# wbuntine/libstb

Measured on AMD Instinct MI355X. Metric: S-table cells/s, higher is better.
Workload: dtype f64

## Files before the change

include/stb_hip.h:

```cpp
#ifndef STB_HIP_H
#define STB_HIP_H

#include <stddef.h>
#include <stdint.h>

#ifdef __cplusplus
extern "C" {
#endif

const char *stb_last_error(void);
int stb_device_count(void);
int stb_device_name(char *buf, int len);

int stb_set_device(int dev);
int stb_get_device(void);
int stb_device_enter(int dev);
void stb_device_leave(int prev);

void *stb_device_malloc(size_t bytes);
void stb_device_free(void *p);
void *stb_host_malloc(size_t bytes);
void stb_host_free(void *p);
void *stb_host_malloc_huge(size_t bytes);
void stb_host_free_huge(void *p);
// ... 158 lines not shown
  double grad, delta;
} stb_modea_info_t;
int stb_groups_aterms_grad(stb_groups_t *g, const double *x_host, int D, double *val_out, double *grad_out);
int stb_groups_modea(stb_groups_t *g, double a_lo, double a_hi, double tol, int rounds_max, double *a_hat, double *curv,
                     stb_modea_info_t *info);
int stb_groups_update_restaurants(stb_groups_t *g, const uint32_t *T, const double *bpar);
int stb_groups_pairs_begin(stb_groups_t *g);
int stb_groups_pairs_put(stb_groups_t *g, const uint32_t *n, const uint16_t *t, uint64_t count, unsigned *maxn, unsigned *maxt);
int stb_groups_pairs_put_ragged(stb_groups_t *g, int I, const int *K, uint32_t *const *n, uint16_t *const *t, unsigned *maxn, unsigned *maxt);
int stb_groups_pairs_commit(stb_groups_t *g, const uint32_t *T, const double *bpar, unsigned N, unsigned M);
int stb_groups_update_pairs(stb_groups_t *g, const uint32_t *nflat, const uint16_t *tflat);
unsigned stb_groups_fallbacks(void);
int stb_grid_shape(unsigned N, unsigned M, int D, int *C_out, int *G_out, int *K_out);
int stb_groups_shape(const stb_groups_t *g, int *I, uint64_t *G, unsigned *N, unsigned *M, int *Dmax);
int stb_groups_last_form(const stb_groups_t *g, int *fused, int *which, int *sparse, int *C, int *R);
int stb_groups_aterms_timed(stb_groups_t *g, const double *x_host, int D, double *out_host,
                            float *ms_fill, float *ms_sweep, float *ms_terms);

int stb_sample_tcounts(const double *d_table, const double *d_S1, unsigned N, unsigned M, double a,
                       const double *d_bpar, int I, const uint64_t *d_koff , const uint32_t *d_n,
                       uint16_t *d_t, uint32_t *d_T, const double *d_h ,
                       uint64_t seed, uint64_t sweep, void *stream);
typedef struct stb_tcounts stb_tcounts_t;
stb_tcounts_t *stb_tcounts_create(int I, const int *K, const uint32_t *nflat, const uint16_t *tflat,
                                  const double *hflat, unsigned M );
int stb_tcounts_set_h(stb_tcounts_t *s, const double *hflat);
int stb_tcounts_sweep(stb_tcounts_t *s, double a, const double *bpar ,
                      uint64_t seed, uint64_t sweep, int nsweeps);
int stb_tcounts_get(stb_tcounts_t *s, uint16_t *t_out, uint32_t *T_out);
int stb_tcounts_to_groups(stb_tcounts_t *s, stb_groups_t *g, const double *bpar );
// ... 74 lines not shown
```

libstb_amd/capi.py:

```python
from __future__ import annotations

import ctypes as C
import os
from functools import lru_cache

import numpy as np

_HERE = os.path.dirname(os.path.abspath(__file__))
LIB_PATH = os.environ.get("STB_LIB_PATH") or os.path.join(_HERE, "lib", "libstb_amd.so")

S_STABLE, S_UVTABLE, S_FLOAT, S_VERBOSE, S_QUITONBOUND, S_THREADS, S_ASYMPT = 1, 2, 4, 8, 16, 32, 64
FILL_SCALED, FILL_LOGDOMAIN, FILL_SCALED_STEP, FILL_SPLIT, FILL_FUSED, FILL_PC, FILL_CHAIN, FILL_CHAINX, FILL_CK, FILL_HB = 0, 1, 2, 3, 4, 5, 6, 7, 8, 9

c_double_p = C.POINTER(C.c_double)
c_u32_p = C.POINTER(C.c_uint32)
c_u16_p = C.POINTER(C.c_uint16)
c_int_p = C.POINTER(C.c_int)
c_float_p = C.POINTER(C.c_float)

LOGDENS = C.CFUNCTYPE(C.c_double, C.c_double, C.c_void_p)
GETVAL = C.CFUNCTYPE(None, c_u32_p, c_u16_p, C.c_uint, C.c_uint)


class StbError(RuntimeError):
# ... 34 lines not shown
    if not os.path.exists(LIB_PATH):
        raise StbError(
            f"{LIB_PATH} is missing: build it with `python -c 'import __graft_entry__ as g; g.build()'` "
            "or `make -C libstb_amd/csrc` (there is no pure-Python or CPU implementation)")
    try:
        import torch
    except Exception:
        pass
    L = C.CDLL(LIB_PATH)
    u, d, i, vp, u64, sz = C.c_uint, C.c_double, C.c_int, C.c_void_p, C.c_uint64, C.c_size_t

    ROUND5 = {"stb_groups_pairs_begin", "stb_groups_pairs_put", "stb_groups_pairs_put_ragged", "stb_groups_pairs_commit",
              "stb_groups_update_pairs", "stb_groups_fallbacks", "stb_grid_shape", "stb_bterms_update",
              "stb_table_probe", "stb_slow_launches", "stb_shared_gpu_mode", "stb_set_shared_gpu", "stb_note_launch_span",
              "stb_lookup_V", "stb_lookup_U", "stb_lookup_UV", "stb_groups_aterms_multi", "stb_groups_create_node",
              "stb_groups_last_form"}

    def sig(name, res, args):
        try:
            f = getattr(L, name)
        except AttributeError:
            if name in ROUND5 and os.environ.get("STB_LIB_PATH"):
                return
            raise
        f.restype = res
        f.argtypes = args

    sig("S_make", vp, [u, u, u, u, d, C.c_uint32])
    sig("S_tag", None, [vp, C.c_char_p])
    sig("S_remake", i, [vp, d])
    sig("S_free", None, [vp])
# ... 65 lines not shown
    sig("stb_groups_aterms_async", i, [vp, c_double_p, i, c_double_p, vp])
    sig("stb_groups_wait", i, [vp])
    sig("stb_groups_aterms_multi", i, [C.POINTER(vp), i, c_double_p, i, c_double_p])
    sig("stb_groups_create_node", i, [i, i, c_int_p, c_u32_p, c_u32_p, c_u16_p, c_double_p, u, u, i, C.POINTER(vp)])
    sig("stb_groups_aterms_device", i, [vp, c_double_p, i, vp, vp])
    sig("stb_groups_update_restaurants", i, [vp, c_u32_p, c_double_p])
    sig("stb_groups_pairs_begin", i, [vp])
    sig("stb_groups_pairs_put", i, [vp, c_u32_p, c_u16_p, u64, C.POINTER(u), C.POINTER(u)])
    sig("stb_groups_pairs_put_ragged", i, [vp, i, c_int_p, vp, vp, C.POINTER(u), C.POINTER(u)])
    sig("stb_groups_pairs_commit", i, [vp, c_u32_p, c_double_p, u, u])
    sig("stb_groups_update_pairs", i, [vp, c_u32_p, c_u16_p])
    sig("stb_groups_fallbacks", C.c_uint, [])
    sig("stb_grid_shape", i, [u, u, i, c_int_p, c_int_p, c_int_p])
    sig("stb_groups_shape", i, [vp, c_int_p, C.POINTER(u64), C.POINTER(u), C.POINTER(u), c_int_p])
    sig("stb_groups_last_form", i, [vp, c_int_p, c_int_p, c_int_p, c_int_p, c_int_p])
    sig("stb_sampler_cache_clear", None, [])
    sig("stb_groups_aterms_timed", i, [vp, c_double_p, i, c_double_p, c_float_p, c_float_p, c_float_p])
    sig("stb_sample_tcounts", i, [vp, vp, u, u, d, vp, i, vp, vp, vp, vp, vp, u64, u64, vp])
    sig("stb_tcounts_create", vp, [i, c_int_p, c_u32_p, c_u16_p, c_double_p, u])
    sig("stb_tcounts_set_h", i, [vp, c_double_p])
    sig("stb_tcounts_sweep", i, [vp, d, c_double_p, u64, u64, i])
    sig("stb_tcounts_get", i, [vp, c_u16_p, c_u32_p])
    sig("stb_tcounts_to_groups", i, [vp, vp, c_double_p])
    sig("stb_tcounts_free", None, [vp])
    sig("stb_sample_tcounts_window", i, [vp, vp, u, u, d, vp, i, vp, vp, vp, vp, vp, u, u, u64, u64, vp])
    sig("stb_tcounts_sweep_window", i, [vp, d, c_double_p, u, u, u64, u64, i])
    sig("stb_sample_tindic", i, [vp, u, u, d, vp, i, vp, vp, vp, vp, vp, vp, vp, u, u64, u64, vp])
    sig("stb_tindic_create", vp, [i, c_int_p, c_u32_p, c_u16_p, c_double_p, c_u32_p, u, u])
    sig("stb_tindic_set_h", i, [vp, c_double_p])
    sig("stb_tindic_sweep", i, [vp, d, c_double_p, u64, u64, i])
# ... 709 lines not shown
```

libstb_amd/csrc/grid_hb.hip:

```cpp
#include <mutex>
#include <vector>

#include "fill_chain.h"

#define GH_PMAX 7
#define GH_NWMAX 8
#define GH_MAXR 48
#define GH_SL 4
#define GH_FSL 4
#define GH_EOFF32 (1u << 30)
#define GH_WRITTEN 0x8000000000000000ull
#define GH_SPIN 48
#define GH_MAXPH 16
#define GH_JOB_MB 192
#define GH_JOBS 1500
#define GH_JQ 64
#define GH_JNUM (GH_JQ + 1)
#define GH_JBASE 128
#define GH_PB(C) ((C) == 8 ? 9 : 8)
#ifndef GH_NOSTORE
#define GH_NOSTORE 0
#endif

struct gh_args {
  const double *a;
  const double2 *lt;
  unsigned *hdr;
  unsigned *ticket;
  unsigned long long *ck_v;
  unsigned *ck_e;
  double *state_v;
  int *state_e;
  const unsigned *tile_off;
  const unsigned *tinfo;
// ... 39 lines not shown
}

template <int C>
__device__ __forceinline__ void gh_row(double (&v)[C], double (&coef)[C], double s) {
  const double t0 = wave_shr1_zero(v[C - 1]) * s;
#pragma unroll
  for (int i = C - 1; i >= 1; i--) v[i] = fma(coef[i], v[i], v[i - 1]);
  v[0] = fma(coef[0], v[0], t0);
#pragma unroll
  for (int i = 0; i < C; i++) coef[i] += 1.0;
}

__host__ __device__ static inline int gh_first_block(int j, int UC, int R) { return (int)(((long long)j * UC) / R); }

template <int C, int K>
__device__ __forceinline__ void gh_lookup(bool valid, unsigned pos, unsigned cnt, const double *stage, const int *se,
                                          const double2 *lt, double a, int mE0, int nrow0, int one_hi, long long &accK, double &accF) {
  static_assert(K == 2 || (K == 4 && C >= 4), "rows between two staged ones");
  constexpr int WS = 64 * C;
  if (valid) {
    const int cw = (int)(pos & ((1u << GH_PB(C)) - 1u)), r = (int)(pos >> GH_PB(C)) & 31;
    const int j = r & (K - 1);
    const double *row = stage + (r / K) * WS;
    const int ln = cw / C;
    const int e = se[ln];
    const int dl = (ln > 0 ? se[ln - 1] : e) - e;
    const double sfac = ldexp(1.0, min(max(dl, -1100), 220));
    const int ci = cw & (C - 1);
    const double c10 = fma(-(double)(mE0 + cw), a, (double)(nrow0 + r - j));
    double x;
    if constexpr (K == 2) {
      const double v0 = row[cw];
      const double v1 = row[cw - 1 < 0 ? 0 : cw - 1] * (ci < 1 ? sfac : 1.0);
      x = j ? fma(c10, v0, v1) : v0;
    } else {
      const double v0 = row[cw];
      const double v1 = row[cw - 1 < 0 ? 0 : cw - 1] * (ci < 1 ? sfac : 1.0);
      const double v2 = row[cw - 2 < 0 ? 0 : cw - 2] * (ci < 2 ? sfac : 1.0);
      const double v3 = row[cw - 3 < 0 ? 0 : cw - 3] * (ci < 3 ? sfac : 1.0);
      const double a2 = a + a;
      const double w0 = fma(c10, v0, v1), w1 = fma(c10 + a, v1, v2), w2 = fma(c10 + a2, v2, v3);
      const double c20 = c10 + 1.0;
      const double u0 = fma(c20, w0, w1), u1 = fma(c20 + a, w1, w2);
      const double t0 = fma(c20 + 1.0, u0, u1);
      x = (j == 0) ? v0 : ((j == 1) ? w0 : ((j == 2) ? u0 : t0));
    }
    const int hi = __double2hiint(x);
    const double2 t = lt[(hi >> 13) & 127];
    const double z = __hiloint2double(mantissa_of_one(hi, one_hi), __double2loint(x));
    const double rr = fma(z, t.x, -1.0);
    double pl = fma(rr, 0.2, -0.25);
    pl = fma(rr, pl, 1.0 / 3.0);
    pl = fma(rr, pl, -0.5);
    pl = fma(rr, pl, 1.0);
    const int kx = (int)((hi >> 20) & 0x7ff) - 1023 + e;
    accK += (long long)(int)cnt * (long long)kx;
    accF = fma((double)cnt, fma(rr, pl, t.y), accF);
  }
}

#ifndef GH_C8_WAVES
#define GH_C8_WAVES 2
#endif
template <int C, int G, int K>
__global__ __launch_bounds__(64 * GH_NWMAX, (C == 8 ? GH_C8_WAVES : 2)) void k_grid_hb(gh_args X) {
  static_assert(C == 2 || C == 4 || C == 8, "columns per lane");
  static_assert(G % K == 0 && G >= K && G <= 32, "rows per group");
  constexpr int WS = 64 * C, SR = G / K;
  constexpr int MHL = GH_MAXR / C;
  constexpr int SL = GH_SL, SLH = SL / 2, FSL = GH_FSL;
  __shared__ double2 lt[128];
  __shared__ __attribute__((aligned(16))) double xv[GH_PMAX][SL][MHL * C];
  __shared__ int xe[GH_PMAX][SL][MHL];
  __shared__ __attribute__((aligned(16))) double fv[FSL][MHL * C];
  __shared__ int fe[FSL][MHL];
  __shared__ int posted[GH_NWMAX], taken[GH_NWMAX], fetched, s_abort, s_awake;
  __shared__ unsigned s_ticket;
  __shared__ int w_se[GH_PMAX][64];
  __shared__ unsigned s_jq[GH_JQ + 1];
  extern __shared__ __attribute__((aligned(16))) double gh_dyn[];

  const int tid = threadIdx.x, lane = tid & 63;
  const int wave = __builtin_amdgcn_readfirstlane(tid >> 6);
  if (tid == 0) s_ticket = atomicAdd(X.ticket, 1u);
  if (tid < 128) lt[tid] = X.lt[tid];
  if (X.jobs && tid <= GH_JQ) s_jq[tid] = X.jobs[tid];
  __syncthreads();
  const unsigned n_jobs = X.jobs ? min((unsigned)__builtin_amdgcn_readfirstlane((int)X.jobs[GH_JNUM]), X.job_cap) : 0u;
  const unsigned ticket = s_ticket;
  if (ticket == 0 && tid == 0) atomicCAS(reinterpret_cast<unsigned long long *>(X.hdr + STB_HDR_T0), 0ull, (unsigned long long)wall_clock64());
  const int R = X.R, HL = X.HL, U = X.U, NB = X.NB, P = X.P;
  const int UC = U * C;
  const int bB = X.b_begin, bE = X.b_end;
// ... 46 lines not shown
    }
    int one_hi = 0x3ff00000;
    asm volatile("" : "+v"(one_hi));
    const bool has_next = (w + 1 < P) && (jw + 1 < X.JWa);
    const int *left_cnt = (w == 0) ? &fetched : &posted[w > 0 ? w - 1 : 0];
    const double *left_v = (w == 0) ? &fv[0][0] : &xv[w > 0 ? w - 1 : 0][0][0];
    const int *left_e = (w == 0) ? &fe[0][0] : &xe[w > 0 ? w - 1 : 0][0][0];
    const int left_mask = (w == 0) ? FSL - 1 : SL - 1;
    unsigned long long *dbg = (X.dbg && d == 0 && lane == 0) ? X.dbg + (size_t)jw * (NB + 2) : nullptr;
    const bool rec = (w == P - 1) && (jw + 1 < X.JWa) && lane >= U;
    const size_t rec_base = ((size_t)d * X.B + j) * (size_t)NB;
    unsigned long long *rec_v = X.ck_v + (rec_base * HL + (lane - U)) * C;
    unsigned *rec_e = X.ck_e + rec_base * HL + (lane - U);
    double s = 1.0;
    double *stage = gh_dyn + (size_t)w * (size_t)(SR * WS);
    int *se = &w_se[w][0];
    const int NQ = R / G;
    long long accK = 0;
    double accF = 0.0;
    auto block_rows = [&](int b, unsigned ti, unsigned &wcur, unsigned tin, size_t item_blk, bool only_walk) {
      {
        const int dl = wave_shr1(ep, ep) - ep;
        s = ldexp(1.0, min(max(dl, -1100), 220));
      }
#pragma unroll
      for (int i = 0; i < C; i++) coef[i] = (double)(1 + b * R) - (double)(m0 + i) * a;
      se[lane] = ep;
      const unsigned nw = ti & 63u;
      const unsigned *tw = X.dense + (size_t)(ti >> 6) * 64 + lane;
      for (int q = 0; q < NQ; q++) {
        const bool listed = !only_walk && ((nw == 63u) || __ballot(wcur != 0) != 0);
        asm volatile("" ::: "memory");
        unsigned wnext = 0;
        if (q + 1 < NQ) {
          if (nw != 0 && nw != 63u) wnext = tw[(size_t)(q + 1) * nw * 64];
        } else {
          tin = (unsigned)__builtin_amdgcn_readfirstlane((int)tin);
          if ((tin & 63u) != 0 && (tin & 63u) != 63u) wnext = X.dense[(size_t)(tin >> 6) * 64 + lane];
        }
        if (listed && !(X.diag & 8)) {
#pragma unroll
          for (int r = 0; r < G; r++) {
// ... 2 lines not shown
              double *dst = stage + (r / K) * WS + lane * C;
#pragma unroll
              for (int i = 0; i < C; i += 2) *reinterpret_cast<gh_double2 *>(dst + i) = gh_double2{v[i], v[i + 1]};
            }
          }
          const int nrow0 = 2 + b * R + q * G;
          if (X.diag & 4) {
          } else if (nw != 63u) {
            const unsigned *gw = tw + (size_t)q * nw * 64;
            unsigned wd = wcur;
            for (unsigned k = 0; k < nw; k++) {
              if (k > 0 && __ballot(wd != 0) == 0) break;
              asm volatile("" ::: "memory");
              unsigned wn = 0;
              if (k + 1 < nw) wn = gw[(size_t)(k + 1) * 64];
              gh_lookup<C, K>(wd != 0, wd & ((1u << (GH_PB(C) + 5)) - 1u), wd >> (GH_PB(C) + 5), stage, se, lt, a, mE0, nrow0, one_hi, accK, accF);
              wd = wn;
            }
          } else {
            const size_t item = item_blk + q;
            const unsigned e0 = X.item_ptr[item], e1 = X.item_ptr[item + 1];
            for (unsigned kk = e0; kk < e1; kk += 64) {
              unsigned pos = 0, cnt = 0;
              if (kk + lane < e1) {
                pos = X.ent_pos[kk + lane];
                cnt = X.ent_cnt[kk + lane];
              }
              gh_lookup<C, K>(kk + lane < e1, pos, cnt, stage, se, lt, a, mE0, nrow0, one_hi, accK, accF);
            }
          }
        } else {
#pragma unroll
          for (int r = 0; r < G; r++) gh_row<C>(v, coef, s);
        }
        wcur = wnext;
      }
    };
    auto sums_out = [&](double *out, bool add) {
      double kd = (double)accK;
#pragma unroll
      for (int o = 32; o >= 1; o >>= 1) {
        kd += __shfl_xor(kd, o);
        accF += __shfl_xor(accF, o);
// ... 406 lines not shown
}

void stb_grid_tile_offsets(const grid_geom &g, std::vector<unsigned> &off) {
  off.assign((size_t)g.JW + 2, 0u);
  const int UC = g.U * g.C;
  unsigned o = 0;
  for (int j = 0; j < g.JW; j++) {
    off[j + 1] = o;
    o += (unsigned)(g.NB - gh_first_block(j, UC, g.R));
  }
  off[0] = o;
}

template <int C, int K>
static int gh_launch(const gh_args &X, int G, unsigned grid, int P, hipStream_t st) {
  const size_t shm = (size_t)P * (size_t)(G / K) * 64 * C * sizeof(double);
  size_t ask = shm;
  if ((int)grid <= stb_cu_count() && ask < 84 * 1024 && stb_env_int("STB_GRID_ALONE", 1)) ask = 84 * 1024;
  const dim3 block(64 * (P + 1));
  switch (G) {
    case 8: STB_LAUNCH_SHM((k_grid_hb<C, 8, K>), dim3(grid), block, ask, st, X); break;
    case 12: STB_LAUNCH_SHM((k_grid_hb<C, 12, K>), dim3(grid), block, ask, st, X); break;
    case 16: STB_LAUNCH_SHM((k_grid_hb<C, 16, K>), dim3(grid), block, ask, st, X); break;
    case 24: STB_LAUNCH_SHM((k_grid_hb<C, 24, K>), dim3(grid), block, ask, st, X); break;
    default: return stb_fail("stb_groups_aterms: no grid kernel for groups of %d rows", G);
  }
  return 0;
}

int stb_launch_grid(fill_args &A, int D, char *ws, size_t ws_left, const dot_request *dot, unsigned **hdr_out, hipStream_t st) {
  const unsigned N = A.N, M = A.M;
// ... 92 lines not shown
```

libstb_amd/csrc/groups.h:

```cpp
#ifndef STB_GROUPS_H
#define STB_GROUPS_H

#include "stb_common.h"

#define STB_TERMS_DMAX 64
#define STB_NLISTS 6
#define GH_JQ_HOST 64
#define STB_WS_FORM 4096

struct slab_info {
  int R, G, NQ, UC, HC;
  int PB;
  unsigned UCp;
  const unsigned *rec_off;
};


struct stb_groups {
  int dev;
  int I;
  uint64_t G;
  unsigned N, M;
  int Dmax;
  uint32_t *d_n, *d_T;
  uint16_t *d_t;
  double *d_bpar;
  double *d_tables, *d_S1, *d_out;
// ... 116 lines not shown
```

libstb_amd/csrc/groups.hip:

```cpp

#include <rocprim/device/device_radix_sort.hpp>
#include <rocprim/device/device_run_length_encode.hpp>
#include <rocprim/device/device_scan.hpp>

#include <algorithm>
#include <atomic>
#include <vector>

#include "stb_common.h"

void stb_grid_tile_offsets(const grid_geom &g, std::vector<unsigned> &off);

#include "groups.h"

__global__ void k_pack_pairs(const uint32_t *n, const uint16_t *t, uint64_t G, uint64_t *key) {
  uint64_t g = (uint64_t)blockIdx.x * blockDim.x + threadIdx.x;
  if (g < G) key[g] = ((uint64_t)n[g] << 16) | t[g];
}
__global__ void k_unpack_pairs(const uint64_t *key, uint64_t G, uint32_t *n, uint16_t *t) {
  uint64_t g = (uint64_t)blockIdx.x * blockDim.x + threadIdx.x;
  if (g < G) {
    n[g] = (uint32_t)(key[g] >> 16);
    t[g] = (uint16_t)(key[g] & 0xffff);
  }
// ... 296 lines not shown
    if (tt >= 2) {
      const unsigned e = tt - 2;
      j = e / (unsigned)H.UC;
      cw = (unsigned)H.HC + (e - j * (unsigned)H.UC);
    }
    const unsigned b = (nn - 2) / (unsigned)H.R, r = (nn - 2) - b * (unsigned)H.R;
    const unsigned b0 = (unsigned)(((unsigned long long)j * (unsigned)H.UC) / (unsigned)H.R);
    const unsigned rec = H.rec_off[j + 1] + (b - b0);
    const unsigned q = r / (unsigned)H.G;
    k = ((((uint64_t)rec * (unsigned)H.NQ) + q) << 11) | ((uint64_t)(r - q * (unsigned)H.G) << 8) | cw;
  }
  key[g] = k;
  payload[g] = (uint32_t)g;
}

__global__ void k_item_keys_hb2(const uint32_t *n, const uint16_t *t, uint64_t G, unsigned N, unsigned M, hb_dot_info H, int posbits,
                                uint64_t *key, uint32_t *payload) {
  const uint64_t g = (uint64_t)blockIdx.x * blockDim.x + threadIdx.x;
  if (g >= G) return;
  const unsigned nn = n[g], tt = t[g];
  uint64_t k;
  if (nn <= 1 || nn == tt) k = STB_KEY_SKIP;
  else if (tt == 0 || nn < tt || tt > M || nn > N) k = STB_KEY_OTHER;
  else {
    unsigned j = 0, cw = (unsigned)H.HC - 1u;
    if (tt >= 2) {
      const unsigned e = tt - 2;
      j = e / (unsigned)H.UC;
      cw = (unsigned)H.HC + (e - j * (unsigned)H.UC);
    }
    const unsigned b = (nn - 2) / (unsigned)H.R, r = (nn - 2) - b * (unsigned)H.R;
    const unsigned b0 = (unsigned)(((unsigned long long)j * (unsigned)H.UC) / (unsigned)H.R);
    const unsigned rec = H.rec_off[j + 1] + (b - b0);
    const unsigned q = r / (unsigned)H.G;
    k = ((((uint64_t)rec * (unsigned)H.NQ) + q) << (posbits + 5)) | ((uint64_t)(r - q * (unsigned)H.G) << posbits) | cw;
  }
  key[g] = k;
  payload[g] = (uint32_t)g;
}

__global__ void k_key_bounds(const uint64_t *key, uint64_t G, uint64_t *counts) {
  if (blockIdx.x != 0 || threadIdx.x != 0) return;
  uint64_t lo = 0, hi = G;
  while (lo < hi) {
    const uint64_t mid = (lo + hi) / 2;
    if (key[mid] < STB_KEY_OTHER) lo = mid + 1;
    else hi = mid;
  }
  const uint64_t a = lo;
  hi = G;
// ... 3 lines not shown
    else hi = mid;
  }
  counts[0] = a;
  counts[1] = lo - a;
}

__global__ void k_gather_pairs(const uint32_t *n, const uint16_t *t, const uint32_t *idx, uint64_t cnt, uint32_t *n2,
                               uint16_t *t2) {
  const uint64_t g = (uint64_t)blockIdx.x * blockDim.x + threadIdx.x;
  if (g < cnt) {
    n2[g] = n[idx[g]];
    t2[g] = t[idx[g]];
  }
}

__global__ void k_split_runs(const uint64_t *ukey, const unsigned *runs, unsigned short *pos, unsigned *item, int posbits) {
  const unsigned r = blockIdx.x * blockDim.x + threadIdx.x;
  if (r < *runs) {
    pos[r] = (unsigned short)(ukey[r] & ((1u << posbits) - 1u));
    item[r] = (unsigned)(ukey[r] >> posbits);
  }
}

#define STB_DENSE_NWMAX 40
#define STB_DENSE_CSR 63u
__global__ void k_tile_words(const unsigned *item_ptr, const unsigned *cnt, unsigned n_tiles, unsigned NQ, int wbits, unsigned *tnw, unsigned *twords) {
  const unsigned t = blockIdx.x * (blockDim.x / 64) + threadIdx.x / 64, lane = threadIdx.x & 63;
  if (t >= n_tiles) return;
  const unsigned e0 = item_ptr[(size_t)t * NQ], e1 = item_ptr[(size_t)t * NQ + NQ];
  unsigned nw = 0;
  for (unsigned q = 0; q < NQ; q++) {
    const unsigned c = item_ptr[(size_t)t * NQ + q + 1] - item_ptr[(size_t)t * NQ + q];
    nw = max(nw, (c + 63) / 64);
  }
  bool big = false;
// ... 250 lines not shown
  uint32_t *p0 = nullptr, *p1 = nullptr;
  unsigned *cnt = nullptr, *runs = nullptr, *item = nullptr;
  void *tmp = nullptr;
  int rc = 1;
  const unsigned blocks = (unsigned)((G + 255) / 256);
  do {
    if (stb_pool_malloc((void **)&k0, 8 * G) != hipSuccess || stb_pool_malloc((void **)&k1, 8 * G) != hipSuccess ||
        stb_pool_malloc((void **)&p0, 4 * G) != hipSuccess || stb_pool_malloc((void **)&p1, 4 * G) != hipSuccess ||
        stb_pool_malloc((void **)&uk, 8 * G) != hipSuccess || stb_pool_malloc((void **)&cnt, 4 * G) != hipSuccess ||
        stb_pool_malloc((void **)&item, 4 * G) != hipSuccess || stb_pool_malloc((void **)&runs, 64) != hipSuccess ||
        stb_pool_malloc((void **)&d_counts, 64) != hipSuccess) {
      stb_fail("stb_groups_aterms: out of device memory");
      break;
    }
    if (which >= 3)
      hipLaunchKernelGGL(k_item_keys_hb2, dim3(blocks), dim3(256), 0, g->st, g->d_n, g->d_t, G, N, M, H, stb_pos_bits(H.C), k0, p0);
    else if (which == 2)
      hipLaunchKernelGGL(k_item_keys_hb, dim3(blocks), dim3(256), 0, g->st, g->d_n, g->d_t, G, N, M, H, k0, p0);
    else
      hipLaunchKernelGGL(k_item_keys, dim3(blocks), dim3(256), 0, g->st, g->d_n, g->d_t, G, N, M, nsg, which ? 2u : 1u, k0, p0);
    size_t b1 = 0, b2 = 0;
    if (rocprim::radix_sort_pairs(nullptr, b1, k0, k1, p0, p1, (size_t)G, 0, 64, g->st) != hipSuccess) break;
    if (rocprim::run_length_encode(nullptr, b2, k1, (unsigned)G, uk, cnt, runs, g->st) != hipSuccess) break;
    const size_t tmp_bytes = b1 > b2 ? b1 : b2;
    if (stb_pool_malloc(&tmp, tmp_bytes ? tmp_bytes : 1) != hipSuccess) {
      stb_fail("stb_groups_aterms: out of device memory");
      break;
    }
    size_t bb = tmp_bytes;
    if (rocprim::radix_sort_pairs(tmp, bb, k0, k1, p0, p1, (size_t)G, 0, 64, g->st) != hipSuccess) break;
    hipLaunchKernelGGL(k_key_bounds, dim3(1), dim3(1), 0, g->st, k1, G, d_counts);
// ... 35 lines not shown
      for (void **q : olds) {
        stb_pool_free(*q);
        *q = nullptr;
      }
      g->ent_cap[which] = 0;
      g->dense_cap[which] = 0;
    }
    if (stb_pool_malloc((void **)&g->d_ent_pos[which], 2 * (size_t)(h_runs ? h_runs : 1)) != hipSuccess ||
        stb_pool_malloc((void **)&g->d_ent_cnt[which], 4 * (size_t)(h_runs ? h_runs : 1)) != hipSuccess ||
        stb_pool_malloc((void **)&g->d_item_ptr[which], 4 * ((size_t)nitems + 2)) != hipSuccess) {
      stb_fail("stb_groups_aterms: out of device memory");
      break;
    }
    if (h_runs) {
      hipLaunchKernelGGL(k_split_runs, dim3((h_runs + 255) / 256), dim3(256), 0, g->st, uk, runs, g->d_ent_pos[which], item,
                         which >= 3 ? stb_pos_bits(H.C) + 5 : (which == 2 ? 11 : 9));
      if (hipMemcpyAsync(g->d_ent_cnt[which], cnt, 4 * (size_t)h_runs, hipMemcpyDeviceToDevice, g->st) != hipSuccess) break;
    }
    hipLaunchKernelGGL(k_item_ptr, dim3((nitems + 1 + 255) / 256), dim3(256), 0, g->st, item, runs, nitems, g->d_item_ptr[which]);
    if (which >= 3) {
      const unsigned n_tiles = H.n_tiles, NQ = (unsigned)H.NQ;
      unsigned *tnw = nullptr, *twords = nullptr, *toff = nullptr;
      void *tmp2 = nullptr;
      size_t b3 = 0;
      bool ok = stb_pool_malloc((void **)&tnw, 4 * (size_t)(n_tiles + 1)) == hipSuccess &&
                stb_pool_malloc((void **)&twords, 4 * (size_t)(n_tiles + 1)) == hipSuccess &&
                stb_pool_malloc((void **)&toff, 4 * (size_t)(n_tiles + 1)) == hipSuccess &&
                stb_pool_malloc((void **)&g->d_tinfo[which], 4 * (size_t)(n_tiles + 1)) == hipSuccess;
      unsigned h_last[2] = {0, 0};
      if (ok && n_tiles) {
        hipLaunchKernelGGL(k_tile_words, dim3((n_tiles + 3) / 4), dim3(256), 0, g->st, g->d_item_ptr[which], g->d_ent_cnt[which], n_tiles, NQ,
// ... 526 lines not shown
  }
  stb_device_leave(prev_dev);
  return rc;
}

extern "C" int stb_groups_last_form(const stb_groups_t *g, int *fused, int *which, int *sparse, int *C_out, int *R_out) {
  if (!g) return 1;
  if (fused) *fused = g->last_fused;
  if (which) *which = g->sel_which;
  if (sparse) *sparse = g->sparse;
  if (C_out) *C_out = g->last_C;
  if (R_out) *R_out = g->last_R;
  return 0;
}

extern "C" int stb_groups_shape(const stb_groups_t *g, int *I, uint64_t *G, unsigned *N, unsigned *M, int *Dmax) {
  if (!g) return 1;
  if (I) *I = g->I;
  if (G) *G = g->G;
  if (N) *N = g->N;
  if (M) *M = g->M;
  if (Dmax) *Dmax = g->Dmax;
  return 0;
}
```

libstb_amd/csrc/lists.hip:

```cpp
#include <rocprim/device/device_scan.hpp>

#include <algorithm>
#include <vector>

#include <pthread.h>
#include <sched.h>

#include "groups.h"

void stb_grid_tile_offsets(const grid_geom &g, std::vector<unsigned> &off);


__device__ __forceinline__ int slab_word(unsigned nn, unsigned tt, unsigned N, unsigned M, const slab_info &H, unsigned &item, size_t &idx) {
  if (nn <= 1 || nn == tt) return 0;
  if (tt == 0 || nn < tt || tt > M || nn > N) return 1;
  unsigned j = 0, col = 0;
  if (tt >= 2) {
    const unsigned e = tt - 2;
    j = e / (unsigned)H.UC;
    col = 1 + (e - j * (unsigned)H.UC);
  }
  const unsigned b = (nn - 2) / (unsigned)H.R, r = (nn - 2) - b * (unsigned)H.R;
  const unsigned b0 = (j * (unsigned)H.UC) / (unsigned)H.R;
  const unsigned rec = H.rec_off[j + 1] + (b - b0);
  const unsigned q = r / (unsigned)H.G;
  item = rec * (unsigned)H.NQ + q;
  idx = ((size_t)item * (unsigned)H.G + (r - q * (unsigned)H.G)) * H.UCp + col;
  return 2;
}

__global__ __launch_bounds__(256) void k_count_cells(const uint32_t *n, const uint16_t *t, uint64_t G, unsigned N, unsigned M, slab_info H,
                                                     unsigned *slab, unsigned long long *ninf) {
  const uint64_t g = (uint64_t)blockIdx.x * blockDim.x + threadIdx.x;
  int kind = 0;
  unsigned item = 0;
  size_t idx = 0;
  if (g < G) kind = slab_word(n[g], t[g], N, M, H, item, idx);
  if (kind == 2) __hip_atomic_fetch_add(&slab[idx], 1u, __ATOMIC_RELAXED, __HIP_MEMORY_SCOPE_AGENT);
  const unsigned long long m = __ballot(kind == 1);
  if (m && (threadIdx.x & 63) == 0) atomicAdd(ninf, (unsigned long long)__popcll(m));
}

// ... 37 lines not shown
      const unsigned cc[4] = {c.x, c.y, c.z, c.w};
      const unsigned mine = (cc[0] != 0u) + (cc[1] != 0u) + (cc[2] != 0u) + (cc[3] != 0u);
      unsigned before = 0, total = 0;
#pragma unroll
      for (int j = 0; j < 4; j++) {
        const unsigned long long m = __ballot(cc[j] != 0u);
        before += (unsigned)__popcll(m & below);
        total += (unsigned)__popcll(m);
      }
      if (mine) {
        unsigned o = out + before;
        bool any = false;
#pragma unroll
        for (int j = 0; j < 4; j++)
          if (cc[j] != 0u) {
            const unsigned ii = i + j, r = ii / H.UCp, col = ii - r * H.UCp;
            ent_pos[o] = (unsigned short)((r << H.PB) | ((unsigned)H.HC - 1u + col));
            ent_cnt[o] = cc[j];
            o++;
            any = true;
          }
        if (any) *reinterpret_cast<uint4 *>(w + i) = uint4{0u, 0u, 0u, 0u};
      }
      out += total;
    }
    return;
  }
  unsigned c0 = (lane < len) ? w[lane] : 0u;
  for (unsigned k = 0; k < len && out < end; k += 64) {
    const unsigned i = k + lane;
    const unsigned c = c0;
    if (k + 64 < len) c0 = (i + 64 < len) ? w[i + 64] : 0u;
    const unsigned long long m = __ballot(c != 0u);
    if (c != 0u) {
      const unsigned o = out + (unsigned)__popcll(m & below);
      const unsigned r = i / H.UCp, col = i - r * H.UCp;
      ent_pos[o] = (unsigned short)((r << H.PB) | ((unsigned)H.HC - 1u + col));
      ent_cnt[o] = c;
      w[i] = 0u;
    }
    out += (unsigned)__popcll(m);
  }
}

#define STB_DENSE_NWMAX 40

__global__ __launch_bounds__(1024) void k_scan_lists(const unsigned *icnt, unsigned nitems, unsigned n_tiles, unsigned NQ, unsigned *item_ptr, unsigned *tnw,
                                                     unsigned *toff, unsigned *tinfo) {
  __shared__ unsigned s_scan[17];
  const unsigned tid = threadIdx.x;
  auto block_exclusive = [&](unsigned mine) -> unsigned { return stb_block_exclusive_1024(mine, s_scan, nullptr); };
  {
// ... 30 lines not shown
                                                   unsigned NQ, int wbits, unsigned *tnw, const unsigned *toff, unsigned *tinfo, unsigned *dense) {
  const unsigned item = blockIdx.x * 4 + (threadIdx.x >> 6), lane = threadIdx.x & 63;
  if (item >= nitems) return;
  const unsigned tile = item / NQ, q = item - tile * NQ;
  const unsigned first = item_ptr[item], end = item_ptr[item + 1];
  const unsigned nw = tinfo[tile] & 63u;
  unsigned *dw = (nw != 0u && nw != 63u) ? dense + ((size_t)toff[tile] + (size_t)q * nw) * 64 : nullptr;
  const unsigned room = nw * 64u;
  if (first != end) {
    unsigned out = first;
    const unsigned len = (unsigned)H.G * H.UCp;
    unsigned *w = slab + (size_t)item * len;
    const unsigned long long below = (1ull << lane) - 1ull;
    const bool wide = (((size_t)item * len) & 3u) == 0 && (len & 3u) == 0;
    auto place = [&](unsigned o, unsigned ii, unsigned c) {
      const unsigned r = ii / H.UCp, col = ii - r * H.UCp;
      const unsigned pos = (r << H.PB) | ((unsigned)H.HC - 1u + col);
      ent_pos[o] = (unsigned short)pos;
      ent_cnt[o] = c;
      if (dw) dw[o - first] = pos | (c << wbits);
      if (c >= (1u << (32 - wbits))) {
        atomicOr(&tinfo[tile], 63u);
        atomicMax(&tnw[tile], 63u);
      }
    };
    if (wide) {
      auto load4 = [&](unsigned i) -> uint4 { return (i + 3 < len) ? *reinterpret_cast<const uint4 *>(w + i) : uint4{0u, 0u, 0u, 0u}; };
      uint4 nx = load4(lane * 4);
      for (unsigned k = 0; k < len && out < end; k += 256) {
        const unsigned i = k + lane * 4;
        const uint4 c = nx;
        if (k + 256 < len) nx = load4(i + 256);
// ... 84 lines not shown
  const uint64_t G = g->G;
  if (G == 0 || G >= 0xffffffffull) return 2;
  if (G * 3 > stb_table_cells(N, M)) return 2;
  slab_info S;
  S.R = H.R;
  S.G = H.G;
  S.NQ = H.NQ;
  S.UC = H.UC;
  S.HC = H.HC;
  S.UCp = (unsigned)H.UC + 1u;
  S.rec_off = H.rec_off;
  const uint64_t nitems64 = (uint64_t)H.n_rec * (unsigned)H.NQ;
  const uint64_t elems64 = nitems64 * (unsigned)H.G * S.UCp;
  if (nitems64 >= (1ull << 31) || elems64 * 4 > slab_limit_bytes()) return 2;
  S.PB = which >= 3 ? stb_pos_bits(H.C) : 8;
  if (H.G > 32 || H.HC - 1 + (int)S.UCp > (1 << S.PB)) return 2;
  if (which >= 3 && (size_t)H.NQ * ((size_t)(g->G / 64) + H.n_tiles + 1) >= (1u << 26)) return 2;
  const unsigned nitems = (unsigned)nitems64;
  const size_t elems = (size_t)elems64;
  hipStream_t st = g->st;
  if (!g->d_slab || g->slab_elems < elems || g->slab_which != which || g->slab_R != H.R || g->slab_G != H.G || g->slab_UCp != (int)S.UCp ||
      g->slab_items != nitems) {
    if (g->d_slab) HIPCHK(hipStreamSynchronize(st));
    if (!g->d_slab || g->slab_elems < elems) {
      FREE_Z(g->d_slab);
      g->slab_elems = 0;
      if (stb_pool_malloc((void **)&g->d_slab, 4 * elems) != hipSuccess) return stb_fail("stb_groups_aterms: out of device memory (count slab, %zu MB)", (4 * elems) >> 20);
      g->slab_elems = elems;
      g->slab_clean = 0;
    }
// ... 420 lines not shown
```

Before: 219.2 billion.

## Sort grid list entries by row-within-stage and skip unused recurrence depth per wave

Entries in each grid item are now ordered by row offset within the staged row group (r mod K), both in the key sort and in the slab layout. This lets a wave-wide ballot pick the deepest recurrence step any lane needs, so the lookup skips the extra loads and FMAs when no lane needs them. The per-lane exponent difference is also precomputed and kept with the exponent as an int2 in dynamic shared memory, which removes a neighbour shared-memory read and clamp from each lookup. The sort key grows by two bits and the slab/list row mapping gains divides and mods. A host-side list-dump API is added for inspection.

Result: no change. 218.7 billion (-0.3%).

```diff
diff --git a/include/stb_hip.h b/include/stb_hip.h
--- a/include/stb_hip.h
+++ b/include/stb_hip.h
@@ -196,6 +196,8 @@
 int stb_grid_shape(unsigned N, unsigned M, int D, int *C_out, int *G_out, int *K_out);
 int stb_groups_shape(const stb_groups_t *g, int *I, uint64_t *G, unsigned *N, unsigned *M, int *Dmax);
 int stb_groups_last_form(const stb_groups_t *g, int *fused, int *which, int *sparse, int *C, int *R);
+int stb_groups_grid_lists(stb_groups_t *g, unsigned *sizes, unsigned *item_ptr, unsigned short *ent_pos, unsigned *ent_cnt,
+                          unsigned *tinfo, unsigned *dense, size_t dense_cap);
 int stb_groups_aterms_timed(stb_groups_t *g, const double *x_host, int D, double *out_host,
                             float *ms_fill, float *ms_sweep, float *ms_terms);
 
diff --git a/libstb_amd/capi.py b/libstb_amd/capi.py
--- a/libstb_amd/capi.py
+++ b/libstb_amd/capi.py
@@ -72,7 +72,7 @@
               "stb_groups_update_pairs", "stb_groups_fallbacks", "stb_grid_shape", "stb_bterms_update",
               "stb_table_probe", "stb_slow_launches", "stb_shared_gpu_mode", "stb_set_shared_gpu", "stb_note_launch_span",
               "stb_lookup_V", "stb_lookup_U", "stb_lookup_UV", "stb_groups_aterms_multi", "stb_groups_create_node",
-              "stb_groups_last_form"}
+              "stb_groups_last_form", "stb_groups_grid_lists"}
 
     def sig(name, res, args):
         try:
@@ -168,6 +168,7 @@
     sig("stb_grid_shape", i, [u, u, i, c_int_p, c_int_p, c_int_p])
     sig("stb_groups_shape", i, [vp, c_int_p, C.POINTER(u64), C.POINTER(u), C.POINTER(u), c_int_p])
     sig("stb_groups_last_form", i, [vp, c_int_p, c_int_p, c_int_p, c_int_p, c_int_p])
+    sig("stb_groups_grid_lists", i, [vp, vp, vp, vp, vp, vp, vp, sz])
     sig("stb_sampler_cache_clear", None, [])
     sig("stb_groups_aterms_timed", i, [vp, c_double_p, i, c_double_p, c_float_p, c_float_p, c_float_p])
     sig("stb_sample_tcounts", i, [vp, vp, u, u, d, vp, i, vp, vp, vp, vp, vp, u64, u64, vp])
diff --git a/libstb_amd/csrc/grid_hb.hip b/libstb_amd/csrc/grid_hb.hip
--- a/libstb_amd/csrc/grid_hb.hip
+++ b/libstb_amd/csrc/grid_hb.hip
@@ -18,6 +18,12 @@
 #define GH_JNUM (GH_JQ + 1)
 #define GH_JBASE 128
 #define GH_PB(C) ((C) == 8 ? 9 : 8)
+#ifndef GH_DEPTH
+#define GH_DEPTH 1
+#endif
+#ifndef GH_STAGED_DL
+#define GH_STAGED_DL 1
+#endif
 #ifndef GH_NOSTORE
 #define GH_NOSTORE 0
 #endif
@@ -87,8 +93,7 @@
 __host__ __device__ static inline int gh_first_block(int j, int UC, int R) { return (int)(((long long)j * UC) / R); }
 
 template <int C, int K>
-__device__ __forceinline__ void gh_lookup(bool valid, unsigned pos, unsigned cnt, const double *stage, const int *se,
-                                          const double2 *lt, double a, int mE0, int nrow0, int one_hi, long long &accK, double &accF) {
+__device__ __forceinline__ void gh_lookup(int depth, bool valid, unsigned pos, unsigned cnt, const double *stage, const int2 *se, const double2 *lt, double a, int mE0, int nrow0, int one_hi, long long &accK, double &accF) {
   static_assert(K == 2 || (K == 4 && C >= 4), "rows between two staged ones");
   constexpr int WS = 64 * C;
   if (valid) {
@@ -96,27 +101,42 @@
     const int j = r & (K - 1);
     const double *row = stage + (r / K) * WS;
     const int ln = cw / C;
-    const int e = se[ln];
-    const int dl = (ln > 0 ? se[ln - 1] : e) - e;
-    const double sfac = ldexp(1.0, min(max(dl, -1100), 220));
+    const int2 ed = se[ln];
+    const int e = ed.x;
     const int ci = cw & (C - 1);
-    const double c10 = fma(-(double)(mE0 + cw), a, (double)(nrow0 + r - j));
-    double x;
-    if constexpr (K == 2) {
-      const double v0 = row[cw];
-      const double v1 = row[cw - 1 < 0 ? 0 : cw - 1] * (ci < 1 ? sfac : 1.0);
-      x = j ? fma(c10, v0, v1) : v0;
-    } else {
-      const double v0 = row[cw];
-      const double v1 = row[cw - 1 < 0 ? 0 : cw - 1] * (ci < 1 ? sfac : 1.0);
-      const double v2 = row[cw - 2 < 0 ? 0 : cw - 2] * (ci < 2 ? sfac : 1.0);
-      const double v3 = row[cw - 3 < 0 ? 0 : cw - 3] * (ci < 3 ? sfac : 1.0);
-      const double a2 = a + a;
-      const double w0 = fma(c10, v0, v1), w1 = fma(c10 + a, v1, v2), w2 = fma(c10 + a2, v2, v3);
-      const double c20 = c10 + 1.0;
-      const double u0 = fma(c20, w0, w1), u1 = fma(c20 + a, w1, w2);
-      const double t0 = fma(c20 + 1.0, u0, u1);
-      x = (j == 0) ? v0 : ((j == 1) ? w0 : ((j == 2) ? u0 : t0));
+    const double v0 = row[cw];
+    double x = v0;
+    if (depth > 0) {
+      const double r1 = row[cw - 1 < 0 ? 0 : cw - 1];
+      double r2 = 0.0, r3 = 0.0;
+      if (K == 4 && depth > 1) r2 = row[cw - 2 < 0 ? 0 : cw - 2];
+      if (K == 4 && depth > 2) r3 = row[cw - 3 < 0 ? 0 : cw - 3];
+      asm volatile("" : "+v"(r2), "+v"(r3));
+#if GH_STAGED_DL
+      const double sfac = ldexp(1.0, ed.y);
+#else
+      const double sfac = ldexp(1.0, min(max((ln > 0 ? se[ln - 1].x : e) - e, -1100), 220));
+#endif
+      const double c10 = fma(-(double)(mE0 + cw), a, (double)(nrow0 + r - j));
+      const double v1 = r1 * (ci < 1 ? sfac : 1.0);
+      const double w0 = fma(c10, v0, v1);
+      if (K == 2 || depth == 1) {
+        x = j ? w0 : v0;
+      } else {
+        const double v2 = r2 * (ci < 2 ? sfac : 1.0);
+        const double w1 = fma(c10 + a, v1, v2);
+        const double c20 = c10 + 1.0;
+        const double u0 = fma(c20, w0, w1);
+        if (depth == 2) {
+          x = (j == 0) ? v0 : ((j == 1) ? w0 : u0);
+        } else {
+          const double v3 = r3 * (ci < 3 ? sfac : 1.0);
+          const double w2 = fma(c10 + (a + a), v2, v3);
+          const double u1 = fma(c20 + a, w1, w2);
+          const double t0 = fma(c20 + 1.0, u0, u1);
+          x = (j == 0) ? v0 : ((j == 1) ? w0 : ((j == 2) ? u0 : t0));
+        }
+      }
     }
     const int hi = __double2hiint(x);
     const double2 t = lt[(hi >> 13) & 127];
@@ -129,6 +149,20 @@
     const int kx = (int)((hi >> 20) & 0x7ff) - 1023 + e;
     accK += (long long)(int)cnt * (long long)kx;
     accF = fma((double)cnt, fma(rr, pl, t.y), accF);
+  }
+}
+
+template <int C, int K>
+__device__ __forceinline__ int gh_depth(unsigned pos) {
+#if !GH_DEPTH
+  return K - 1;
+#endif
+  const unsigned jj = (pos >> GH_PB(C)) & (unsigned)(K - 1);
+  if constexpr (K == 2) {
+    return __ballot(jj != 0) != 0 ? 1 : 0;
+  } else {
+    if (__ballot(jj >= 2) != 0) return __ballot(jj == 3) != 0 ? 3 : 2;
+    return __ballot(jj != 0) != 0 ? 1 : 0;
   }
 }
 
@@ -149,7 +183,6 @@
   __shared__ int fe[FSL][MHL];
   __shared__ int posted[GH_NWMAX], taken[GH_NWMAX], fetched, s_abort, s_awake;
   __shared__ unsigned s_ticket;
-  __shared__ int w_se[GH_PMAX][64];
   __shared__ unsigned s_jq[GH_JQ + 1];
   extern __shared__ __attribute__((aligned(16))) double gh_dyn[];
 
@@ -226,18 +259,19 @@
     unsigned *rec_e = X.ck_e + rec_base * HL + (lane - U);
     double s = 1.0;
     double *stage = gh_dyn + (size_t)w * (size_t)(SR * WS);
-    int *se = &w_se[w][0];
+    int2 *se = reinterpret_cast<int2 *>(gh_dyn + (size_t)P * (size_t)(SR * WS)) + w * 64;
     const int NQ = R / G;
     long long accK = 0;
     double accF = 0.0;
     auto block_rows = [&](int b, unsigned ti, unsigned &wcur, unsigned tin, size_t item_blk, bool only_walk) {
+      int dl;
       {
-        const int dl = wave_shr1(ep, ep) - ep;
-        s = ldexp(1.0, min(max(dl, -1100), 220));
+        dl = min(max(wave_shr1(ep, ep) - ep, -1100), 220);
+        s = ldexp(1.0, dl);
       }
 #pragma unroll
       for (int i = 0; i < C; i++) coef[i] = (double)(1 + b * R) - (double)(m0 + i) * a;
-      se[lane] = ep;
+      se[lane] = make_int2(ep, dl);
       const unsigned nw = ti & 63u;
       const unsigned *tw = X.dense + (size_t)(ti >> 6) * 64 + lane;
       for (int q = 0; q < NQ; q++) {
@@ -270,7 +304,8 @@
               asm volatile("" ::: "memory");
               unsigned wn = 0;
               if (k + 1 < nw) wn = gw[(size_t)(k + 1) * 64];
-              gh_lookup<C, K>(wd != 0, wd & ((1u << (GH_PB(C) + 5)) - 1u), wd >> (GH_PB(C) + 5), stage, se, lt, a, mE0, nrow0, one_hi, accK, accF);
+              gh_lookup<C, K>(gh_depth<C, K>(wd), wd != 0, wd & ((1u << (GH_PB(C) + 5)) - 1u), wd >> (GH_PB(C) + 5), stage, se, lt, a, mE0, nrow0, one_hi,
+                              accK, accF);
               wd = wn;
             }
           } else {
@@ -282,7 +317,7 @@
                 pos = X.ent_pos[kk + lane];
                 cnt = X.ent_cnt[kk + lane];
               }
-              gh_lookup<C, K>(kk + lane < e1, pos, cnt, stage, se, lt, a, mE0, nrow0, one_hi, accK, accF);
+              gh_lookup<C, K>(gh_depth<C, K>(pos), kk + lane < e1, pos, cnt, stage, se, lt, a, mE0, nrow0, one_hi, accK, accF);
             }
           }
         } else {
@@ -719,7 +754,7 @@
 
 template <int C, int K>
 static int gh_launch(const gh_args &X, int G, unsigned grid, int P, hipStream_t st) {
-  const size_t shm = (size_t)P * (size_t)(G / K) * 64 * C * sizeof(double);
+  const size_t shm = (size_t)P * (size_t)(G / K) * 64 * C * sizeof(double) + (size_t)P * 64 * sizeof(int2);
   size_t ask = shm;
   if ((int)grid <= stb_cu_count() && ask < 84 * 1024 && stb_env_int("STB_GRID_ALONE", 1)) ask = 84 * 1024;
   const dim3 block(64 * (P + 1));
diff --git a/libstb_amd/csrc/groups.h b/libstb_amd/csrc/groups.h
--- a/libstb_amd/csrc/groups.h
+++ b/libstb_amd/csrc/groups.h
@@ -11,6 +11,7 @@
 struct slab_info {
   int R, G, NQ, UC, HC;
   int PB;
+  int K;
   unsigned UCp;
   const unsigned *rec_off;
 };
diff --git a/libstb_amd/csrc/groups.hip b/libstb_amd/csrc/groups.hip
--- a/libstb_amd/csrc/groups.hip
+++ b/libstb_amd/csrc/groups.hip
@@ -334,7 +334,8 @@
   payload[g] = (uint32_t)g;
 }
 
-__global__ void k_item_keys_hb2(const uint32_t *n, const uint16_t *t, uint64_t G, unsigned N, unsigned M, hb_dot_info H, int posbits,
+#define STB_KEY_DEPTH_BITS 2
+__global__ void k_item_keys_hb2(const uint32_t *n, const uint16_t *t, uint64_t G, unsigned N, unsigned M, hb_dot_info H, int posbits, unsigned K,
                                 uint64_t *key, uint32_t *payload) {
   const uint64_t g = (uint64_t)blockIdx.x * blockDim.x + threadIdx.x;
   if (g >= G) return;
@@ -353,7 +354,8 @@
     const unsigned b0 = (unsigned)(((unsigned long long)j * (unsigned)H.UC) / (unsigned)H.R);
     const unsigned rec = H.rec_off[j + 1] + (b - b0);
     const unsigned q = r / (unsigned)H.G;
-    k = ((((uint64_t)rec * (unsigned)H.NQ) + q) << (posbits + 5)) | ((uint64_t)(r - q * (unsigned)H.G) << posbits) | cw;
+    const unsigned rg = r - q * (unsigned)H.G;
+    k = ((((uint64_t)rec * (unsigned)H.NQ) + q) << (posbits + 5 + STB_KEY_DEPTH_BITS)) | ((uint64_t)(rg % K) << (posbits + 5)) | ((uint64_t)rg << posbits) | cw;
   }
   key[g] = k;
   payload[g] = (uint32_t)g;
@@ -387,11 +389,11 @@
   }
 }
 
-__global__ void k_split_runs(const uint64_t *ukey, const unsigned *runs, unsigned short *pos, unsigned *item, int posbits) {
+__global__ void k_split_runs(const uint64_t *ukey, const unsigned *runs, unsigned short *pos, unsigned *item, int posbits, int skip) {
   const unsigned r = blockIdx.x * blockDim.x + threadIdx.x;
   if (r < *runs) {
     pos[r] = (unsigned short)(ukey[r] & ((1u << posbits) - 1u));
-    item[r] = (unsigned)(ukey[r] >> posbits);
+    item[r] = (unsigned)(ukey[r] >> (posbits + skip));
   }
 }
 
@@ -672,7 +674,8 @@
       break;
     }
     if (which >= 3)
-      hipLaunchKernelGGL(k_item_keys_hb2, dim3(blocks), dim3(256), 0, g->st, g->d_n, g->d_t, G, N, M, H, stb_pos_bits(H.C), k0, p0);
+      hipLaunchKernelGGL(k_item_keys_hb2, dim3(blocks), dim3(256), 0, g->st, g->d_n, g->d_t, G, N, M, H, stb_pos_bits(H.C),
+                         (unsigned)((gg.K > 1 && H.G % gg.K == 0) ? gg.K : 1), k0, p0);
     else if (which == 2)
       hipLaunchKernelGGL(k_item_keys_hb, dim3(blocks), dim3(256), 0, g->st, g->d_n, g->d_t, G, N, M, H, k0, p0);
     else
@@ -738,7 +741,7 @@
     }
     if (h_runs) {
       hipLaunchKernelGGL(k_split_runs, dim3((h_runs + 255) / 256), dim3(256), 0, g->st, uk, runs, g->d_ent_pos[which], item,
-                         which >= 3 ? stb_pos_bits(H.C) + 5 : (which == 2 ? 11 : 9));
+                         which >= 3 ? stb_pos_bits(H.C) + 5 : (which == 2 ? 11 : 9), which >= 3 ? STB_KEY_DEPTH_BITS : 0);
       if (hipMemcpyAsync(g->d_ent_cnt[which], cnt, 4 * (size_t)h_runs, hipMemcpyDeviceToDevice, g->st) != hipSuccess) break;
     }
     hipLaunchKernelGGL(k_item_ptr, dim3((nitems + 1 + 255) / 256), dim3(256), 0, g->st, item, runs, nitems, g->d_item_ptr[which]);
@@ -1295,6 +1298,48 @@
   return 0;
 }
 
+extern "C" int stb_groups_grid_lists(stb_groups_t *g, unsigned *sizes, unsigned *item_ptr, unsigned short *ent_pos, unsigned *ent_cnt, unsigned *tinfo,
+                                     unsigned *dense, size_t dense_cap) {
+  STB_ENTRY;
+  if (!g || !sizes) return stb_fail("stb_groups_grid_lists: null argument");
+  const int which = g->sel_which;
+  if (which < 3 || which >= STB_NLISTS || !g->lists_ready[which] || !g->d_tile_off[which] || !g->d_tinfo[which])
+    return stb_fail("stb_groups_grid_lists: the set's last evaluation did not take the grid form");
+  const int prev = stb_device_enter(g->dev);
+  int rc = 1;
+  do {
+    if (hipStreamSynchronize(g->st) != hipSuccess) break;
+    unsigned n_tiles = 0, n_ent = 0;
+    if (hipMemcpy(&n_tiles, g->d_tile_off[which], 4, hipMemcpyDeviceToHost) != hipSuccess) break;
+    const unsigned NQ = (unsigned)(g->list_R[which] / g->list_G[which]), nitems = n_tiles * NQ;
+    if (hipMemcpy(&n_ent, g->d_item_ptr[which] + nitems, 4, hipMemcpyDeviceToHost) != hipSuccess) break;
+    std::vector<unsigned> ti(n_tiles);
+    if (n_tiles && hipMemcpy(ti.data(), g->d_tinfo[which], 4 * (size_t)n_tiles, hipMemcpyDeviceToHost) != hipSuccess) break;
+    size_t words = 0;
+    for (unsigned t : ti)
+      if ((t & 63u) != 0u && (t & 63u) != 63u) words = std::max(words, (size_t)(t >> 6) + (size_t)(t & 63u) * NQ);
+    sizes[0] = n_tiles;
+    sizes[1] = NQ;
+    sizes[2] = n_ent;
+    sizes[3] = (unsigned)words;
+    if (item_ptr && hipMemcpy(item_ptr, g->d_item_ptr[which], 4 * ((size_t)nitems + 1), hipMemcpyDeviceToHost) != hipSuccess) break;
+    if (ent_pos && n_ent && hipMemcpy(ent_pos, g->d_ent_pos[which], 2 * (size_t)n_ent, hipMemcpyDeviceToHost) != hipSuccess) break;
+    if (ent_cnt && n_ent && hipMemcpy(ent_cnt, g->d_ent_cnt[which], 4 * (size_t)n_ent, hipMemcpyDeviceToHost) != hipSuccess) break;
+    if (tinfo && n_tiles) memcpy(tinfo, ti.data(), 4 * (size_t)n_tiles);
+    if (dense && words) {
+      if (dense_cap < words * 64) {
+        stb_fail("stb_groups_grid_lists: room for %zu dense words, %zu in use", dense_cap, words * 64);
+        break;
+      }
+      if (hipMemcpy(dense, g->d_dense[which], 256 * words, hipMemcpyDeviceToHost) != hipSuccess) break;
+    }
+    rc = 0;
+  } while (0);
+  if (rc && hipGetLastError() != hipSuccess) stb_fail("stb_groups_grid_lists: a copy from the device failed");
+  stb_device_leave(prev);
+  return rc;
+}
+
 extern "C" int stb_groups_shape(const stb_groups_t *g, int *I, uint64_t *G, unsigned *N, unsigned *M, int *Dmax) {
   if (!g) return 1;
   if (I) *I = g->I;
diff --git a/libstb_amd/csrc/lists.hip b/libstb_amd/csrc/lists.hip
--- a/libstb_amd/csrc/lists.hip
+++ b/libstb_amd/csrc/lists.hip
@@ -10,6 +10,12 @@
 
 void stb_grid_tile_offsets(const grid_geom &g, std::vector<unsigned> &off);
 
+
+__device__ __forceinline__ unsigned slab_row(unsigned r, const slab_info &H) { return (r % (unsigned)H.K) * ((unsigned)H.G / (unsigned)H.K) + r / (unsigned)H.K; }
+__device__ __forceinline__ unsigned list_row(unsigned rp, const slab_info &H) {
+  const unsigned sr = (unsigned)H.G / (unsigned)H.K;
+  return (rp % sr) * (unsigned)H.K + rp / sr;
+}
 
 __device__ __forceinline__ int slab_word(unsigned nn, unsigned tt, unsigned N, unsigned M, const slab_info &H, unsigned &item, size_t &idx) {
   if (nn <= 1 || nn == tt) return 0;
@@ -25,7 +31,7 @@
   const unsigned rec = H.rec_off[j + 1] + (b - b0);
   const unsigned q = r / (unsigned)H.G;
   item = rec * (unsigned)H.NQ + q;
-  idx = ((size_t)item * (unsigned)H.G + (r - q * (unsigned)H.G)) * H.UCp + col;
+  idx = ((size_t)item * (unsigned)H.G + slab_row(r - q * (unsigned)H.G, H)) * H.UCp + col;
   return 2;
 }
 
@@ -93,8 +99,8 @@
 #pragma unroll
         for (int j = 0; j < 4; j++)
           if (cc[j] != 0u) {
-            const unsigned ii = i + j, r = ii / H.UCp, col = ii - r * H.UCp;
-            ent_pos[o] = (unsigned short)((r << H.PB) | ((unsigned)H.HC - 1u + col));
+            const unsigned ii = i + j, rp = ii / H.UCp, col = ii - rp * H.UCp;
+            ent_pos[o] = (unsigned short)((list_row(rp, H) << H.PB) | ((unsigned)H.HC - 1u + col));
             ent_cnt[o] = cc[j];
             o++;
             any = true;
@@ -113,8 +119,8 @@
     const unsigned long long m = __ballot(c != 0u);
     if (c != 0u) {
       const unsigned o = out + (unsigned)__popcll(m & below);
-      const unsigned r = i / H.UCp, col = i - r * H.UCp;
-      ent_pos[o] = (unsigned short)((r << H.PB) | ((unsigned)H.HC - 1u + col));
+      const unsigned rp = i / H.UCp, col = i - rp * H.UCp;
+      ent_pos[o] = (unsigned short)((list_row(rp, H) << H.PB) | ((unsigned)H.HC - 1u + col));
       ent_cnt[o] = c;
       w[i] = 0u;
     }
@@ -175,8 +181,8 @@
     const unsigned long long below = (1ull << lane) - 1ull;
     const bool wide = (((size_t)item * len) & 3u) == 0 && (len & 3u) == 0;
     auto place = [&](unsigned o, unsigned ii, unsigned c) {
-      const unsigned r = ii / H.UCp, col = ii - r * H.UCp;
-      const unsigned pos = (r << H.PB) | ((unsigned)H.HC - 1u + col);
+      const unsigned rp = ii / H.UCp, col = ii - rp * H.UCp;
+      const unsigned pos = (list_row(rp, H) << H.PB) | ((unsigned)H.HC - 1u + col);
       ent_pos[o] = (unsigned short)pos;
       ent_cnt[o] = c;
       if (dw) dw[o - first] = pos | (c << wbits);
@@ -291,6 +297,7 @@
   const uint64_t elems64 = nitems64 * (unsigned)H.G * S.UCp;
   if (nitems64 >= (1ull << 31) || elems64 * 4 > slab_limit_bytes()) return 2;
   S.PB = which >= 3 ? stb_pos_bits(H.C) : 8;
+  S.K = (which >= 3 && gg.K > 1 && H.G % gg.K == 0) ? gg.K : 1;
   if (H.G > 32 || H.HC - 1 + (int)S.UCp > (1 << S.PB)) return 2;
   if (which >= 3 && (size_t)H.NQ * ((size_t)(g->G / 64) + H.n_tiles + 1) >= (1u << 26)) return 2;
   const unsigned nitems = (unsigned)nitems64;
```
